# MartinMikkelsen/TensorTrainNumerics.jl

Measured on AMD Instinct MI355X. Metric: TT cores/sec for QTT Laplacian apply+round, d=30 rank-64, higher is better.
Workload: dtype f64

## Files before the change

tensortrainnumerics.jl_amd/csrc/ttn_eig_kernels.h:

```cpp
#pragma once
#include "ttn_wg_gemm.h"
#include "ttn_wg_jacobi.h"

#define EIG_N 128
template <int J>
__device__ __forceinline__ void fmac_bcast(double& a, double w, double s_) {
    asm volatile("v_fmac_f64_dpp %0, %1, %2 row_newbcast:%3 row_mask:0xf bank_mask:0xf" : "+v"(a) : "v"(w), "v"(s_), "n"(J));
}
#define EIG_BCAST16(M) M(0) M(1) M(2) M(3) M(4) M(5) M(6) M(7) M(8) M(9) M(10) M(11) M(12) M(13) M(14) M(15)
#define EIG_TAIL TTN_LDS_IMG

__device__ __forceinline__ void lds_barrier() { asm volatile("s_waitcnt lgkmcnt(0)\n\ts_barrier" ::: "memory"); }
__device__ __forceinline__ double wave64_sum_mfma(double v) {
    v = grp_sum(v);
    v += dpp_mov_f64<0x124>(v);
    v += dpp_mov_f64<0x128>(v);
    return v;
}
__device__ __forceinline__ double readlane_f64(double v, int idx) {
    union { double d; int i[2]; } u, r;
    u.d = v;
    r.i[0] = __builtin_amdgcn_readlane(u.i[0], idx);
    r.i[1] = __builtin_amdgcn_readlane(u.i[1], idx);
    return r.d;
}

template <int N>
__device__ __noinline__ void wg_tridiag(const double* Gg, int ldg, double* Vst, double* lds) {
    Gg = unip(Gg); Vst = unip(Vst); lds = unip(lds); ldg = uni32(ldg);
    constexpr bool TWO = (N == 128);
    constexpr int CW = (N * N / 16 > TTN_WG) ? 32 : 16;
    constexpr int NH = CW / 16;
    constexpr int NC = N / CW;
    static_assert(N * NC <= TTN_WG, "one thread per (row, column chunk)");
    lds_f64* L = (lds_f64*)lds;
    lds_f64 *vbuf0 = L, *vbuf1 = L + 128, *wL = L + 256, *xnext = L + 384, *part = L + 512;
    lds_f64 *dg = L + EIG_TAIL, *e = dg + 128, *beta = dg + 384;
    const int tid = threadIdx.x, lane = tid & 63, wave = tid >> 6;
    const int i = tid & (N - 1), c = tid / N;
    const bool actv = tid < N * NC;
    double a[CW];
#pragma unroll
    for (int j = 0; j < CW; ++j) a[j] = actv ? Gg[i + (long long)ldg * (CW * c + j)] : 0.0;
    lds_f64* xt = L + 1664;
    if (actv && i == 0) {
#pragma unroll
        for (int j = 0; j < CW; ++j) wL[CW * c + j] = a[j];
    }
    if (actv && i == 1) {
#pragma unroll
        for (int j = 0; j < CW; ++j) xnext[CW * c + j] = a[j];
    }
    __syncthreads();
    double rx0 = 0.0, rx1 = 0.0, ralpha = 0.0, rden = 0.0, rdg = 0.0;
    if (wave == 0) {
        rx0 = (lane > 0) ? wL[lane] : 0.0; rx1 = TWO ? wL[lane + 64] : 0.0;
        const double xk1 = wL[1];
        rdg = wL[0];
        xt[lane] = rx0; xt[lane + 64] = rx1;
        const double s2 = wave64_sum_mfma(fma(rx0, rx0, rx1 * rx1));
        ralpha = (s2 > 0.0) ? -copysign(s2 * fast_rsqrt2(s2), xk1) : 0.0;
        rden = s2 - ralpha * xk1;
    }
    for (int k = 0; k < N - 2; ++k) {
        lds_f64* vL = (k & 1) ? vbuf1 : vbuf0;
        lds_barrier();
        const bool live = actv && (CW * (c + 1) > k + 1) && ((TWO ? 64 * (wave & 1) : 0) + 63 > k);
        double v0 = 0.0, v1 = 0.0, w0 = 0.0, w1 = 0.0, bta = 0.0;
        if (wave == 0) {
            __builtin_amdgcn_s_setprio(TTN_TRIDIAG_PRIO);
            if (rden > 0.0) { bta = fast_rcp(rden); bta = fma(fma(-rden, bta, 1.0), bta, bta); }
            v0 = rx0 - ((lane == k + 1) ? ralpha : 0.0); v1 = rx1 - ((lane + 64 == k + 1) ? ralpha : 0.0);
            vL[lane] = v0; vL[lane + 64] = v1;
            typedef __attribute__((address_space(1))) double gdouble;
            gdouble* vg = (gdouble*)(unsigned long long)(Vst + k * 128);
            vg[lane] = v0; vg[lane + 64] = v1;
            if (lane == 0) { dg[k] = rdg; e[k] = ralpha; beta[k] = bta; }
        }
        if (live) {
            double xreg[NH];
#pragma unroll
            for (int h = 0; h < NH; ++h) xreg[h] = xt[CW * c + 16 * h + (lane & 15)];
            double pp = 0.0;
            asm volatile("s_nop 1");
#define EIG_MV(j) fmac_bcast<j>(pp, xreg[0], a[j]);
            EIG_BCAST16(EIG_MV)
#undef EIG_MV
            if constexpr (NH == 2) {
#define EIG_MV(j) fmac_bcast<j>(pp, xreg[1], a[16 + j]);
                EIG_BCAST16(EIG_MV)
#undef EIG_MV
            }
            part[c * 128 + i] = pp;
        } else if (actv) part[c * 128 + i] = 0.0;
        lds_barrier();
        lds_f64* xn_r = (k & 1) ? xnext + 1152 : xnext;
        lds_f64* xn_w = (k & 1) ? xnext : xnext + 1152;
        if (wave == 0) {
            double p0 = 0.0, p1 = 0.0;
#pragma unroll
            for (int cc = 0; cc < NC; ++cc) { p0 += part[cc * 128 + lane]; if (TWO) p1 += part[cc * 128 + lane + 64]; }
            p0 = bta * fma(-ralpha, xn_r[lane], p0); p1 = TWO ? bta * fma(-ralpha, xn_r[lane + 64], p1) : 0.0;
            const double Kc = 0.5 * bta * wave64_sum_mfma(fma(p0, v0, p1 * v1));
            w0 = fma(-Kc, v0, p0); w1 = fma(-Kc, v1, p1);
            wL[lane] = w0; if (TWO) wL[lane + 64] = w1;
        }
        lds_barrier();
        if (wave == 0 && k + 1 < N - 2) {
            const double wk1 = wL[k + 1], vk1 = vL[k + 1];
            const double c0 = fma(-v0, wk1, fma(-w0, vk1, xn_r[lane]));
            const double c1 = TWO ? fma(-v1, wk1, fma(-w1, vk1, xn_r[lane + 64])) : 0.0;
            const int kk = k + 1;
            rdg = (kk < 64) ? readlane_f64(c0, kk) : readlane_f64(c1, kk - 64);
            const double xk1 = (kk + 1 < 64) ? readlane_f64(c0, kk + 1) : readlane_f64(c1, kk + 1 - 64);
            rx0 = (lane > kk) ? c0 : 0.0; rx1 = (TWO && lane + 64 > kk) ? c1 : 0.0;
            xt[lane] = rx0; xt[lane + 64] = rx1;
            const double s2 = wave64_sum_mfma(fma(rx0, rx0, rx1 * rx1));
            ralpha = (s2 > 0.0) ? -copysign(s2 * fast_rsqrt2(s2), xk1) : 0.0;
            rden = s2 - ralpha * xk1;
        }
        if (wave == 0) __builtin_amdgcn_s_setprio(TTN_EIG_PRIO);
        if (live) {
            double vreg[NH], wreg[NH];
#pragma unroll
            for (int h = 0; h < NH; ++h) { vreg[h] = vL[CW * c + 16 * h + (lane & 15)]; wreg[h] = wL[CW * c + 16 * h + (lane & 15)]; }
            const double nvi = -vL[i], nwi = -wL[i];
            asm volatile("s_nop 1");
#define EIG_UP(j) fmac_bcast<j>(a[j], wreg[0], nvi); fmac_bcast<j>(a[j], vreg[0], nwi);
            EIG_BCAST16(EIG_UP)
#undef EIG_UP
            if constexpr (NH == 2) {
#define EIG_UP(j) fmac_bcast<j>(a[16 + j], wreg[1], nvi); fmac_bcast<j>(a[16 + j], vreg[1], nwi);
                EIG_BCAST16(EIG_UP)
#undef EIG_UP
            }
            if (i == k + 2) {
#pragma unroll
                for (int j = 0; j < CW; ++j) xn_w[CW * c + j] = a[j];
            }
        }
    }
    __syncthreads();
    if (actv && i == N - 2 && c == NC - 1) { dg[N - 2] = a[CW - 2]; e[N - 2] = a[CW - 1]; }
    if (actv && i == N - 1 && c == NC - 1) { dg[N - 1] = a[CW - 1]; }
    __syncthreads();
}

template <int N>
__device__ __forceinline__ int sturm_count(const double (&dreg)[N / 16], const double (&ereg)[N / 16], double x, bool& zero) {
    double pc = 1.0, pp = 0.0;
    const double nx = -x, one = 1.0;
    int cnt = 0;
    bool z = false;
    unsigned int prev = 0;
#pragma unroll
    for (int g = 0; g < N / 16; ++g) {
        unsigned int bits = 0;
#define EIG_ST(j) {                                                                                               \
            double dmx = nx;                                                                                      \
            fmac_bcast<j>(dmx, dreg[g], one);                                         \
            double pn = dmx * pc;                                                                                 \
            fmac_bcast<j>(pn, ereg[g], pp);                        \
            z |= (pn == 0.0);                                                                                     \
            bits = __builtin_amdgcn_alignbit(bits, (unsigned int)(__double_as_longlong(pn) >> 32), 31);           \
            pp = pc; pc = pn; }
        EIG_BCAST16(EIG_ST)
#undef EIG_ST
        const unsigned int seq = (prev << 16) | (bits & 0xffffu);
        cnt += __popc((seq ^ (seq >> 1)) & 0xffffu);
        prev = bits & 1u;
        const double ap = fabs(pc);
        if (ap < 0x1p-400 || ap > 0x1p400) {
            const double sc = (ap < 1.0) ? 0x1p500 : 0x1p-500;
            pc *= sc; pp *= sc;
        }
    }
    zero = z;
    return cnt;
}
__device__ __noinline__ int sturm_count_guarded(const lds_f64* de, double x, int n) {
    double pc = 1.0, pp = 0.0;
    int cnt = 0;
    for (int i = 0; i < n; ++i) {
        double pn = fma(de[2 * i] - x, pc, de[2 * i + 1] * pp);
        if (pn == 0.0) pn = copysign(DBL_MIN, -pc);
        cnt += (int)(((unsigned long long)(__double_as_longlong(pn) ^ __double_as_longlong(pc))) >> 63);
        pp = pc; pc = pn;
        const double ap = fabs(pc);
        if (ap < 0x1p-400 || ap > 0x1p400) { const double sc = (ap < 1.0) ? 0x1p500 : 0x1p-500; pc *= sc; pp *= sc; }
    }
    return cnt;
}

template <int N, int TL>
__device__ void wg_bisect(int nev, double* lds) {
    lds_f64* L = (lds_f64*)lds;
    lds_f64 *dg = L + EIG_TAIL, *e = dg + 128, *lam = dg + 256;
    lds_f64* e2 = L;
    const int tid = threadIdx.x;
    lds_f64* de = L + 256;
    for (int t = tid; t < N; t += TTN_WG) { e2[t] = (t < N - 1) ? e[t] * e[t] : 0.0; de[2 * t] = dg[t]; de[2 * t + 1] = (t > 0) ? -(e[t - 1] * e[t - 1]) : 0.0; }
    __syncthreads();
    if (tid < 64) {
        double glo_ = 1e300, ghi_ = -1e300, emax_ = 0.0;
        for (int t = tid; t < N; t += 64) {
            const double rad = ((t > 0) ? fabs(e[t - 1]) : 0.0) + ((t < N - 1) ? fabs(e[t]) : 0.0);
            glo_ = fmin(glo_, dg[t] - rad); ghi_ = fmax(ghi_, dg[t] + rad);
            emax_ = fmax(emax_, e2[t]);
        }
        glo_ = -wave_max(-glo_); ghi_ = wave_max(ghi_); emax_ = wave_max(emax_);
        if (tid == 0) { e2[128] = glo_; e2[129] = ghi_; e2[130] = emax_; }
    }
    __syncthreads();
    double glo = e2[128], ghi = e2[129];
    const double emax = e2[130];
    const double span = fmax(fabs(glo), fabs(ghi));
    glo -= 2.0 * DBL_EPSILON * span * N; ghi += 2.0 * DBL_EPSILON * span * N;
    const double pivmin = DBL_MIN * fmax(1.0, emax);
    double dreg[N / 16], ereg[N / 16];
#pragma unroll
    for (int g = 0; g < N / 16; ++g) { dreg[g] = de[2 * (16 * g + (tid & 15))]; ereg[g] = de[2 * (16 * g + (tid & 15)) + 1]; }
    asm volatile("s_nop 1");
    for (int g0 = 0; g0 < nev; g0 += TTN_WG / TL) {
        const int gi = g0 + tid / TL, sub = tid % TL;
        const bool act = gi < nev;
        const int jasc = N - 1 - (act ? gi : 0);
        double lo = glo, hi = ghi;
        for (int round = 0; round < 64; ++round) {
            const double wdt = hi - lo;
            const bool done = !(wdt > 2.0 * DBL_EPSILON * fmax(fabs(lo), fabs(hi)) + 2.0 * pivmin);
            if (__syncthreads_and(done || !act)) break;
            const double x = lo + wdt * ((double)(sub + 1) / (double)(TL + 1));
            const bool wave_act = g0 + (tid & ~63) / TL < nev;
            bool zero = false;
            int cnt = wave_act ? sturm_count<N>(dreg, ereg, x, zero) : 0;
            if (zero) cnt = sturm_count_guarded(de, x, N);
            int nf = (cnt <= jasc) ? 1 : 0;
#pragma unroll
            for (int m = 1; m < TL; m <<= 1) nf += __shfl_xor(nf, m);
            if (!done) {
                const double nlo = (nf > 0) ? lo + wdt * ((double)nf / (double)(TL + 1)) : lo;
                const double nhi = (nf < TL) ? lo + wdt * ((double)(nf + 1) / (double)(TL + 1)) : hi;
                lo = nlo; hi = nhi;
            }
        }
        if (act && sub == 0) lam[gi] = 0.5 * (lo + hi);
    }
    __syncthreads();
}

template <int N>
struct EigDm {
    static constexpr bool IN_LDS = 2 * N * 64 <= TTN_LDS_IMG;
    typedef __attribute__((address_space(1))) double gdouble;
    lds_f64* l;
    gdouble* g;
    __device__ __forceinline__ double ld(int idx) const { if constexpr (IN_LDS) return l[idx]; else return g[idx]; }
    __device__ __forceinline__ void st(int idx, double v) const { if constexpr (IN_LDS) l[idx] = v; else g[idx] = v; }
};
template <int N>
__device__ void wg_twisted(int r, double* lds, int* tw , lds_f64* zn , double* Dmg) {
    lds_f64* L = (lds_f64*)lds;
    lds_f64 *dg = L + EIG_TAIL, *e = dg + 128, *lam = dg + 256;
    lds_f64* Dp = L;
    EigDm<N> Dm;
    Dm.l = L + N * 64; Dm.g = (typename EigDm<N>::gdouble*)(unsigned long long)Dmg;
    const int tid = threadIdx.x, lane = tid & 63, wave = tid >> 6;
    double emax = 0.0;
    for (int t = 0; t < N - 1; ++t) emax = fmax(emax, e[t] * e[t]);
    const double pivmin = DBL_MIN * fmax(1.0, emax);
    __syncthreads();
    const bool act = lane < r;
    const double lm = lam[act ? lane : 0];
    if (wave == 0) {
        double q = 1.0;
        for (int i0 = 0; i0 < N; i0 += 8) {
            double dd[8], ee[8];
#pragma unroll
            for (int t = 0; t < 8; ++t) { dd[t] = dg[i0 + t]; ee[t] = (i0 + t > 0) ? e[i0 + t - 1] : 0.0; }
#pragma unroll
            for (int t = 0; t < 8; ++t) {
                q = fma(-(ee[t] * ee[t]), fast_rcp(q), dd[t] - lm);
                if (fabs(q) < pivmin) q = -pivmin;
                Dp[(i0 + t) * 64 + lane] = q;
            }
        }
    } else if (wave == 1) {
        double q = 1.0;
        for (int i0 = N - 8; i0 >= 0; i0 -= 8) {
            double dd[8], ee[8];
#pragma unroll
            for (int t = 0; t < 8; ++t) { dd[t] = dg[i0 + t]; ee[t] = (i0 + t < N - 1) ? e[i0 + t] : 0.0; }
#pragma unroll
            for (int t = 7; t >= 0; --t) {
                q = fma(-(ee[t] * ee[t]), fast_rcp(q), dd[t] - lm);
                if (fabs(q) < pivmin) q = -pivmin;
                Dm.st((i0 + t) * 64 + lane, q);
            }
        }
    }
    __syncthreads();
    if (wave < 2) {
        double gbest = 1e300;
        int kb = 0;
        for (int i0 = 0; i0 < N; i0 += 8) {
            double dm[8];
#pragma unroll
            for (int t = 0; t < 8; ++t) dm[t] = Dm.ld((i0 + t) * 64 + lane);
#pragma unroll
            for (int t = 0; t < 8; ++t) {
                const double g = fabs(Dp[(i0 + t) * 64 + lane] + dm[t] - (dg[i0 + t] - lm));
                if (g < gbest) { gbest = g; kb = i0 + t; }
            }
        }
        double z = 1.0, nrm = 0.0;
        if (wave == 0) {
            for (int i = kb - 1; i >= 0; --i) {
                z = -(e[i] * fast_rcp(Dp[i * 64 + lane])) * z;
                Dp[i * 64 + lane] = z;
                nrm = fma(z, z, nrm);
            }
            if (act) { tw[lane] = kb; zn[lane] = nrm; }
        } else {
            if constexpr (EigDm<N>::IN_LDS) {
                for (int i = kb; i < N - 1; ++i) {
                    z = -(e[i] * fast_rcp(Dm.ld((i + 1) * 64 + lane))) * z;
                    Dm.st((i + 1) * 64 + lane, z);
                    nrm = fma(z, z, nrm);
                }
            } else {
                for (int i0 = 0; i0 < N - 1; i0 += 8) {
                    double dm[8];
#pragma unroll
                    for (int t = 0; t < 8; ++t) dm[t] = (i0 + t + 1 < N) ? Dm.ld((i0 + t + 1) * 64 + lane) : 1.0;
#pragma unroll
                    for (int t = 0; t < 8; ++t) {
                        const int i = i0 + t;
                        if (i >= kb && i < N - 1) {
                            z = -(e[i] * fast_rcp(dm[t])) * z;
                            Dm.st((i + 1) * 64 + lane, z);
                            nrm = fma(z, z, nrm);
                        }
                    }
                }
            }
            if (act) zn[64 + lane] = nrm;
        }
    }
    __syncthreads();
    if (tid < 64 && tid < r) zn[tid] = 1.0 / sqrt(1.0 + zn[tid] + zn[64 + tid]);
    __syncthreads();
}

template <int N>
__device__ __noinline__ int wg_eig_n(const double* Gg, int ldg, double* Vst, int r, int nev, double* sig, double* lds, int* iwork ,
                                     double* dwork ) {
    Gg = unip(Gg); Vst = unip(Vst); sig = unip(sig); lds = unip(lds); iwork = unip(iwork); dwork = unip(dwork);
    r = uni32(r); nev = uni32(nev); ldg = uni32(ldg);
    constexpr int RPL = N / 16;
    lds_f64* L = (lds_f64*)lds;
    lds_f64 *lam = L + EIG_TAIL + 256, *beta = L + EIG_TAIL + 384;
    const int tid = threadIdx.x, lane = tid & 63, wave = tid >> 6;
    __builtin_amdgcn_s_setprio(TTN_EIG_PRIO);
    wg_tridiag<N>(Gg, ldg, Vst, lds);
    if (nev <= 32) wg_bisect<N, 8>(nev, lds);
    else wg_bisect<N, 4>(nev, lds);
    int bad = 0;
    for (int j = tid; j < nev; j += TTN_WG) { const double l = lam[j]; sig[j] = (l > 0.0) ? sqrt(l) : 0.0; bad |= (j < r) && !(l > 0.0); }
    if (__syncthreads_or(bad)) {
        __builtin_amdgcn_s_setprio(0); TTN_SETPRIO_BASE();
        return 1;
    }
    wg_twisted<N>(r, lds, iwork, (lds_f64*)dwork, const_cast<double*>(Gg));
    lds_f64* Dp = L;
    EigDm<N> Dm;
    Dm.l = L + N * 64; Dm.g = (typename EigDm<N>::gdouble*)(unsigned long long)Gg;
    const int rc = (lane & 3) | ((lane >> 4) << 2), col0 = 8 * (wave & 7) + 2 * ((lane >> 2) & 3);
    double z[2][RPL];
#pragma unroll
    for (int cc = 0; cc < 2; ++cc) {
        const int col = col0 + cc;
        const int kb = (col < r) ? iwork[col] : 0;
        const double zn = (col < r) ? ((lds_f64*)dwork)[col] : 0.0;
#pragma unroll
        for (int t = 0; t < RPL; ++t) {
            const int row = RPL * rc + t;
            const double v = (row < kb) ? Dp[row * 64 + col] : ((row == kb) ? 1.0 : Dm.ld(row * 64 + col));
            z[cc][t] = v * zn;
        }
    }
    constexpr int VROWS = TTN_LDS_IMG / 128;
    for (int khi = N - 2; khi > 0; khi -= VROWS) {
    const int klo = (khi > VROWS) ? khi - VROWS : 0;
    __syncthreads();
    wg_batched<8>((long long)(khi - klo) * 128, [&](long long e_) { return Vst[klo * 128 + e_]; }, [&](long long e_, double v) { L[e_] = v; });
    __syncthreads();
    if (wave < 8) {
        typedef double __attribute__((ext_vector_type(2))) d2;
        typedef __attribute__((address_space(3))) d2 lds_d2;
        for (int k = khi - 1; k >= klo; --k) {
            const lds_d2* vp = (const lds_d2*)(L + (k - klo) * 128 + RPL * rc);
            double vk[RPL];
#pragma unroll
            for (int t = 0; t < RPL / 2; ++t) { const d2 w2 = vp[t]; vk[2 * t] = w2.x; vk[2 * t + 1] = w2.y; }
            const double bk = beta[k];
            double s0 = 0.0, s1 = 0.0;
#pragma unroll
            for (int t = 0; t < RPL; ++t) { s0 = fma(vk[t], z[0][t], s0); s1 = fma(vk[t], z[1][t], s1); }
            const double t0 = grp_sum(s0) * bk, t1 = grp_sum(s1) * bk;
#pragma unroll
            for (int t = 0; t < RPL; ++t) { z[0][t] = fma(-t0, vk[t], z[0][t]); z[1][t] = fma(-t1, vk[t], z[1][t]); }
        }
    }
    }
    __syncthreads();
    if (wave < 8) {
#pragma unroll
        for (int cc = 0; cc < 2; ++cc) {
            const int col = col0 + cc;
            if (col < r) {
                const double sg = sig[col];
#pragma unroll
                for (int t = 0; t < RPL; ++t) L[col * 128 + RPL * rc + t] = z[cc][t] * sg;
            }
        }
    }
    __syncthreads();
    __builtin_amdgcn_s_setprio(0); TTN_SETPRIO_BASE();
    return 0;
}
__device__ int wg_eig128(const double* Gg, double* Vst, int r, int nev, double* sig, double* lds, int* iwork, double* dwork) {
    return wg_eig_n<128>(Gg, 128, Vst, r, nev, sig, lds, iwork, dwork);
}
__device__ int wg_eig64(const double* Gg, int ldg, double* Vst, int r, int nev, double* sig, double* lds, int* iwork, double* dwork) {
    return wg_eig_n<64>(Gg, ldg, Vst, r, nev, sig, lds, iwork, dwork);
}

__global__ void TTN_KERNEL_BOUNDS k_selftest_eig128(const double* G, double* Vst, int n, int r, int nev, double* sig, double* Xout, long long* clk) {
    extern __shared__ double lds[];
    int* iwork = reinterpret_cast<int*>(lds + GEMM_LDS_TOTAL + 32);
    double* dwork = lds + GEMM_LDS_TOTAL + 32 + 64;
    const long long t0 = (long long)__builtin_amdgcn_s_memtime();
    const int rc = (n == 64) ? wg_eig_n<64>(G, 64, Vst, r, nev, sig, lds, iwork, dwork) : wg_eig_n<128>(G, 128, Vst, r, nev, sig, lds, iwork, dwork);
    const long long t1 = (long long)__builtin_amdgcn_s_memtime();
    if (threadIdx.x == 0) { clk[0] = t1 - t0; clk[1] = rc; }
    if (rc == 0) for (int e = threadIdx.x; e < 128 * r; e += TTN_WG) Xout[e] = lds[e];
}
```

Measured before the change: 653,400.

## Keep twisted-factorization backward pivots in registers across holder waves, single LDS array

The backward (Dm) factorization in the twisted eigenvector solver was written to a second LDS array, or to global memory when it did not fit (N=128). Now four holder waves each recompute the backward recurrence and keep their own chunk of pivots in registers. Each holder finds its local best twist index, the candidates are reduced through a small LDS table, and only the rows below the twist are merged into the single LDS array. It also reuses emax computed during bisection instead of recomputing it serially. The aim is to remove global-memory traffic and halve LDS use, at the cost of redundant recurrence work per holder and more register pressure.

```diff
diff --git a/tensortrainnumerics.jl_amd/csrc/ttn_eig_kernels.h b/tensortrainnumerics.jl_amd/csrc/ttn_eig_kernels.h
--- a/tensortrainnumerics.jl_amd/csrc/ttn_eig_kernels.h
+++ b/tensortrainnumerics.jl_amd/csrc/ttn_eig_kernels.h
@@ -209,7 +209,7 @@
             emax_ = fmax(emax_, e2[t]);
         }
         glo_ = -wave_max(-glo_); ghi_ = wave_max(ghi_); emax_ = wave_max(emax_);
-        if (tid == 0) { e2[128] = glo_; e2[129] = ghi_; e2[130] = emax_; }
+        if (tid == 0) { e2[128] = glo_; e2[129] = ghi_; e2[130] = emax_; e[N - 1] = emax_; }
     }
     __syncthreads();
     double glo = e2[128], ghi = e2[129];
@@ -249,29 +249,25 @@
     __syncthreads();
 }
 
+#define EIG_HOLDERS 4
 template <int N>
-struct EigDm {
-    static constexpr bool IN_LDS = 2 * N * 64 <= TTN_LDS_IMG;
-    typedef __attribute__((address_space(1))) double gdouble;
-    lds_f64* l;
-    gdouble* g;
-    __device__ __forceinline__ double ld(int idx) const { if constexpr (IN_LDS) return l[idx]; else return g[idx]; }
-    __device__ __forceinline__ void st(int idx, double v) const { if constexpr (IN_LDS) l[idx] = v; else g[idx] = v; }
-};
-template <int N>
-__device__ void wg_twisted(int r, double* lds, int* tw , lds_f64* zn , double* Dmg) {
+__device__ void wg_twisted(int r, double* lds, int* tw , lds_f64* zn ) {
+    static_assert(N % (8 * EIG_HOLDERS) == 0 && TTN_WG >= 64 * (EIG_HOLDERS + 1) && N * 64 <= TTN_LDS_IMG, "one array in the image; wave 0 and the holders");
+    static_assert(EIG_HOLDERS * 64 + EIG_HOLDERS * 32 <= GEMM_TAB_ENTRIES, "the twist candidates fit the table area");
+    constexpr int HC = N / 8 / EIG_HOLDERS;
     lds_f64* L = (lds_f64*)lds;
     lds_f64 *dg = L + EIG_TAIL, *e = dg + 128, *lam = dg + 256;
-    lds_f64* Dp = L;
-    EigDm<N> Dm;
-    Dm.l = L + N * 64; Dm.g = (typename EigDm<N>::gdouble*)(unsigned long long)Dmg;
-    const int tid = threadIdx.x, lane = tid & 63, wave = tid >> 6;
-    double emax = 0.0;
-    for (int t = 0; t < N - 1; ++t) emax = fmax(emax, e[t] * e[t]);
-    const double pivmin = DBL_MIN * fmax(1.0, emax);
+    lds_f64* D = L;
+    lds_f64* cg = L + GEMM_LDS_DOUBLES + 32;
+    lds_i32* ck = (lds_i32*)(cg + EIG_HOLDERS * 64);
+    const int tid = threadIdx.x, lane = tid & 63, wave = uni32(tid >> 6);
+    const bool holder = wave >= 1 && wave <= EIG_HOLDERS;
+    const int c0 = HC * (wave - 1);
+    const double pivmin = DBL_MIN * fmax(1.0, e[N - 1]);
     __syncthreads();
     const bool act = lane < r;
     const double lm = lam[act ? lane : 0];
+    double keep[HC][8];
     if (wave == 0) {
         double q = 1.0;
         for (int i0 = 0; i0 < N; i0 += 8) {
@@ -282,67 +278,80 @@
             for (int t = 0; t < 8; ++t) {
                 q = fma(-(ee[t] * ee[t]), fast_rcp(q), dd[t] - lm);
                 if (fabs(q) < pivmin) q = -pivmin;
-                Dp[(i0 + t) * 64 + lane] = q;
-            }
-        }
-    } else if (wave == 1) {
-        double q = 1.0;
-        for (int i0 = N - 8; i0 >= 0; i0 -= 8) {
+                D[(i0 + t) * 64 + lane] = q;
+            }
+        }
+    } else if (holder) {
+        auto chunk = [&](int i0, double& q, auto put) {
             double dd[8], ee[8];
 #pragma unroll
-            for (int t = 0; t < 8; ++t) { dd[t] = dg[i0 + t]; ee[t] = (i0 + t < N - 1) ? e[i0 + t] : 0.0; }
+            for (int t = 7; t >= 0; --t) { dd[t] = dg[i0 + t]; ee[t] = (i0 + t < N - 1) ? e[i0 + t] : 0.0; }
 #pragma unroll
             for (int t = 7; t >= 0; --t) {
                 q = fma(-(ee[t] * ee[t]), fast_rcp(q), dd[t] - lm);
                 if (fabs(q) < pivmin) q = -pivmin;
-                Dm.st((i0 + t) * 64 + lane, q);
-            }
-        }
-    }
-    __syncthreads();
+                put(t, q);
+            }
+        };
+        double q = 1.0;
+        for (int ch = N / 8 - 1; ch >= c0 + HC; --ch) chunk(8 * ch, q, [](int, double) {});
+#pragma unroll
+        for (int c = HC - 1; c >= 0; --c) chunk(8 * (c0 + c), q, [&](int t, double v) { keep[c][t] = v; });
+    }
+    lds_barrier();
+    if (holder) {
+        double gbest = 1e300;
+        int kc = 0;
+#pragma unroll
+        for (int c = 0; c < HC; ++c) {
+            const int i0 = 8 * (c0 + c);
+            double dp[8], dd[8];
+#pragma unroll
+            for (int t = 0; t < 8; ++t) { dp[t] = D[(i0 + t) * 64 + lane]; dd[t] = dg[i0 + t]; }
+#pragma unroll
+            for (int t = 0; t < 8; ++t) {
+                const double g = fabs(dp[t] + keep[c][t] - (dd[t] - lm));
+                if (g < gbest) { gbest = g; kc = i0 + t; }
+            }
+        }
+        cg[(wave - 1) * 64 + lane] = gbest; ck[(wave - 1) * 64 + lane] = kc;
+    }
+    lds_barrier();
+    int kb = 0;
+    if (wave <= EIG_HOLDERS) {
+        double gbest = 1e300;
+#pragma unroll
+        for (int h = 0; h < EIG_HOLDERS; ++h) {
+            const double g = cg[h * 64 + lane];
+            const int k = ck[h * 64 + lane];
+            if (g < gbest) { gbest = g; kb = k; }
+        }
+    }
+    if (holder) {
+#pragma unroll
+        for (int c = 0; c < HC; ++c) {
+#pragma unroll
+            for (int t = 0; t < 8; ++t) {
+                const int row = 8 * (c0 + c) + t;
+                if (row > kb) D[row * 64 + lane] = keep[c][t];
+            }
+        }
+    }
+    lds_barrier();
     if (wave < 2) {
-        double gbest = 1e300;
-        int kb = 0;
-        for (int i0 = 0; i0 < N; i0 += 8) {
-            double dm[8];
-#pragma unroll
-            for (int t = 0; t < 8; ++t) dm[t] = Dm.ld((i0 + t) * 64 + lane);
-#pragma unroll
-            for (int t = 0; t < 8; ++t) {
-                const double g = fabs(Dp[(i0 + t) * 64 + lane] + dm[t] - (dg[i0 + t] - lm));
-                if (g < gbest) { gbest = g; kb = i0 + t; }
-            }
-        }
         double z = 1.0, nrm = 0.0;
         if (wave == 0) {
             for (int i = kb - 1; i >= 0; --i) {
-                z = -(e[i] * fast_rcp(Dp[i * 64 + lane])) * z;
-                Dp[i * 64 + lane] = z;
+                z = -(e[i] * fast_rcp(D[i * 64 + lane])) * z;
+                D[i * 64 + lane] = z;
                 nrm = fma(z, z, nrm);
             }
             if (act) { tw[lane] = kb; zn[lane] = nrm; }
         } else {
-            if constexpr (EigDm<N>::IN_LDS) {
-                for (int i = kb; i < N - 1; ++i) {
-                    z = -(e[i] * fast_rcp(Dm.ld((i + 1) * 64 + lane))) * z;
-                    Dm.st((i + 1) * 64 + lane, z);
-                    nrm = fma(z, z, nrm);
-                }
-            } else {
-                for (int i0 = 0; i0 < N - 1; i0 += 8) {
-                    double dm[8];
-#pragma unroll
-                    for (int t = 0; t < 8; ++t) dm[t] = (i0 + t + 1 < N) ? Dm.ld((i0 + t + 1) * 64 + lane) : 1.0;
-#pragma unroll
-                    for (int t = 0; t < 8; ++t) {
-                        const int i = i0 + t;
-                        if (i >= kb && i < N - 1) {
-                            z = -(e[i] * fast_rcp(dm[t])) * z;
-                            Dm.st((i + 1) * 64 + lane, z);
-                            nrm = fma(z, z, nrm);
-                        }
-                    }
-                }
+            for (int i = kb; i < N - 1; ++i) {
+                z = -(e[i] * fast_rcp(D[(i + 1) * 64 + lane])) * z;
+                D[(i + 1) * 64 + lane] = z;
+                nrm = fma(z, z, nrm);
             }
             if (act) zn[64 + lane] = nrm;
         }
@@ -371,10 +380,8 @@
         __builtin_amdgcn_s_setprio(0); TTN_SETPRIO_BASE();
         return 1;
     }
-    wg_twisted<N>(r, lds, iwork, (lds_f64*)dwork, const_cast<double*>(Gg));
-    lds_f64* Dp = L;
-    EigDm<N> Dm;
-    Dm.l = L + N * 64; Dm.g = (typename EigDm<N>::gdouble*)(unsigned long long)Gg;
+    wg_twisted<N>(r, lds, iwork, (lds_f64*)dwork);
+    lds_f64* D = L;
     const int rc = (lane & 3) | ((lane >> 4) << 2), col0 = 8 * (wave & 7) + 2 * ((lane >> 2) & 3);
     double z[2][RPL];
 #pragma unroll
@@ -385,7 +392,7 @@
 #pragma unroll
         for (int t = 0; t < RPL; ++t) {
             const int row = RPL * rc + t;
-            const double v = (row < kb) ? Dp[row * 64 + col] : ((row == kb) ? 1.0 : Dm.ld(row * 64 + col));
+            const double v = (row == kb) ? 1.0 : D[row * 64 + col];
             z[cc][t] = v * zn;
         }
     }
```

New measurement: 668,400 (median of 6 runs). 1.02x the previous value.
